# zju3dv/pats

Measured on AMD Instinct MI355X. Metric: image-pairs/sec (coarse+fine OT) on 640x480 MegaDepth; OT iters/sec per pair, higher is better.
Workload: dtype f32 (contractions: fp32 operands split into fp16 hi + lo, three exact-product MFMA passes, fp32 accumulate)

## Files before the change

### include/pats_amd.h

```cpp
#ifndef PATS_AMD_H
#define PATS_AMD_H

#include <stddef.h>
#include <stdint.h>

#ifdef __cplusplus
extern "C" {
#endif

typedef void* pats_stream_t;

enum {
    PATS_OK = 0,
    PATS_ERR_INVALID = 1,
    PATS_ERR_UNSUPPORTED = 2,
    PATS_ERR_LAUNCH = 3,
    PATS_ERR_NO_DEVICE = 4
};

enum { PATS_SINKHORN_AUTO = 0, PATS_SINKHORN_LOG = 1, PATS_SINKHORN_KERNEL = 2 };

const char* pats_version(void);
#define PATS_ABI_VERSION 8
int pats_abi_version(void);
const char* pats_last_error(void);
int pats_device_count(void);
int pats_set_sinkhorn_mode(int mode);
int pats_set_fine_fused(int on);

int pats_set_third_gather(int mode);

int pats_sinkhorn_fallbacks(int64_t* count, int reset);

int pats_sinkhorn_tail_solves(int64_t* count, int reset);

int pats_cost_f32(const float* d0, const float* d1, int64_t batch, int D, int n, int m, float* out,
                  pats_stream_t stream);

size_t pats_sinkhorn_workspace_bytes(int64_t batch, int M, int N);
int pats_sinkhorn_f32(const float* Z, int64_t batch, int M, int N, const float* log_mu,
                      const float* log_nu, int iters, float* out, void* workspace,
                      size_t workspace_bytes, pats_stream_t stream);

size_t pats_ot_workspace_bytes(int64_t batch, int M, int N);
int pats_log_optimal_transport_f32(const float* scores, int64_t batch, int m, int n,
                                   const float* alpha, const float* ns, int iters, float* Z,
                                   void* workspace, size_t workspace_bytes, pats_stream_t stream);

size_t pats_ot2_workspace_bytes(int64_t batch, int m, int n);
int pats_log_optimal_transport2_flags_f32(const float* scores, int64_t batch, int m, int n,
                                          const float* one, const float* ns, int iters, float bias_k,
                                          float* Z, uint8_t* col_nomatch, void* workspace,
                                          size_t workspace_bytes, pats_stream_t stream);
int pats_log_optimal_transport2_f32(const float* scores, int64_t batch, int m, int n,
                                    const float* one, const float* ns, int iters, float bias_k,
                                    float* Z, void* workspace, size_t workspace_bytes,
                                    pats_stream_t stream);

int pats_cost_ot_f32(const float* d0, const float* d1, int64_t batch, int D, int n, int m,
                     int variant, const float* scalar, const float* ns, int iters, float bias_k,
                     float* Z, void* workspace, size_t workspace_bytes, pats_stream_t stream);
size_t pats_cost_ot_workspace_bytes(int64_t batch, int D, int n, int m, int variant);
int pats_cost_ot_flags_f32(const float* d0, const float* d1, int64_t batch, int D, int n, int m,
// ... 589 lines not shown
```

### pats_amd/_lib.py

```python
import ctypes
import os

_HERE = os.path.dirname(os.path.abspath(__file__))
LIB_PATH = os.path.join(_HERE, "libpats_amd.so")
if os.environ.get("PATS_AMD_DIAG_LIB", "") not in ("", "0"):
    _sfx = os.environ["PATS_AMD_DIAG_LIB"]
    LIB_PATH = os.path.join(_HERE, "libpats_amd_diag%s.so" % ("" if _sfx == "1" else _sfx))

c_void_p, c_int, c_i64, c_f, c_size = (ctypes.c_void_p, ctypes.c_int, ctypes.c_int64, ctypes.c_float,
                                       ctypes.c_size_t)

ABI_VERSION = 8



class PairTable(ctypes.Structure):
    _fields_ = [("pairs", ctypes.c_int64), ("shape_host", c_void_p), ("cell_base_host", c_void_p), ("shape", c_void_p),
                ("cell_base", c_void_p), ("img_base", c_void_p)]


_TAB = ctypes.POINTER(PairTable)


class CropFormat(ctypes.Structure):
    _fields_ = [("dtype", ctypes.c_int32), ("layout", ctypes.c_int32), ("normalize", ctypes.c_int32),
                ("mean", ctypes.c_float * 3), ("std", ctypes.c_float * 3)]


_FMT = ctypes.POINTER(CropFormat)

_SCORE_ARGS = [c_void_p, c_void_p, c_void_p, c_void_p, c_i64, c_void_p, c_i64, c_i64, c_void_p, c_i64, c_void_p, c_void_p, c_int, c_f,
               c_void_p, c_void_p, c_void_p, c_void_p, c_void_p, c_void_p, c_size, c_void_p]
_ADAPTIVE_ARGS = [ctypes.c_double, c_int, c_int, c_i64, c_void_p, c_void_p]
_POLISH_ARGS = [c_void_p, c_void_p, c_void_p, c_void_p, c_i64, c_void_p, c_i64, c_i64, c_void_p, c_void_p, c_int, c_f, c_void_p, c_i64,
                c_void_p, c_int, c_void_p, c_void_p, c_void_p, c_void_p, c_void_p, c_void_p, c_void_p, c_size, c_void_p]

SIGNATURES = {
    "pats_version": (ctypes.c_char_p, []),
    "pats_abi_version": (c_int, []),
    "pats_last_error": (ctypes.c_char_p, []),
    "pats_device_count": (c_int, []),
    "pats_set_sinkhorn_mode": (c_int, [c_int]),
    "pats_set_fine_fused": (c_int, [c_int]),
    "pats_set_third_gather": (c_int, [c_int]),
    "pats_sinkhorn_fallbacks": (c_int, [ctypes.POINTER(ctypes.c_int64), c_int]),
    "pats_sinkhorn_tail_solves": (c_int, [ctypes.POINTER(ctypes.c_int64), c_int]),
    "pats_set_gnn_redo_mode": (c_int, [c_int]),
    "pats_gnn_overflows": (c_int, [ctypes.POINTER(ctypes.c_int64), c_int]),
    "pats_cost_f32": (c_int, [c_void_p, c_void_p, c_i64, c_int, c_int, c_int, c_void_p, c_void_p]),
    "pats_sinkhorn_workspace_bytes": (c_size, [c_i64, c_int, c_int]),
    "pats_sinkhorn_f32": (c_int, [c_void_p, c_i64, c_int, c_int, c_void_p, c_void_p, c_int, c_void_p,
                                  c_void_p, c_size, c_void_p]),
    "pats_ot_workspace_bytes": (c_size, [c_i64, c_int, c_int]),
    "pats_log_optimal_transport_f32": (c_int, [c_void_p, c_i64, c_int, c_int, c_void_p, c_void_p, c_int,
                                               c_void_p, c_void_p, c_size, c_void_p]),
    "pats_ot2_workspace_bytes": (c_size, [c_i64, c_int, c_int]),
    "pats_log_optimal_transport2_f32": (c_int, [c_void_p, c_i64, c_int, c_int, c_void_p, c_void_p, c_int,
                                                c_f, c_void_p, c_void_p, c_size, c_void_p]),
    "pats_cost_ot_f32": (c_int, [c_void_p, c_void_p, c_i64, c_int, c_int, c_int, c_int, c_void_p,
                                 c_void_p, c_int, c_f, c_void_p, c_void_p, c_size, c_void_p]),
    "pats_cost_ot_flags_f32": (c_int, [c_void_p, c_void_p, c_i64, c_int, c_int, c_int, c_int, c_void_p,
                                       c_void_p, c_int, c_f, c_void_p, c_void_p, c_void_p, c_size, c_void_p]),
    "pats_set_cost_ot_mid_event": (c_int, [c_void_p]),
    "pats_cost_ot_flags_counted_f32": (c_int, [c_void_p, c_void_p, c_i64, c_void_p, c_int, c_int, c_int, c_int, c_void_p,
                                               c_void_p, c_int, c_f, c_void_p, c_void_p, c_void_p, c_size, c_void_p]),
    "pats_iterative_expand_counted_f32": (c_int, [c_void_p, c_int, c_i64, c_void_p, c_int, c_int, c_void_p, c_void_p, c_int,
                                                  c_int, c_int, c_f, c_int, c_void_p, c_void_p, c_void_p,
                                                  c_void_p, c_void_p, c_void_p, c_void_p, c_void_p]),
    "pats_fine_descriptors_counted_f32": (c_int, [c_void_p, c_void_p, c_void_p, c_void_p, c_void_p, c_i64, c_void_p, c_int,
                                                  c_void_p, c_void_p]),
    "pats_log_optimal_transport2_flags_f32": (c_int, [c_void_p, c_i64, c_int, c_int, c_void_p, c_void_p, c_int,
                                                      c_f, c_void_p, c_void_p, c_void_p, c_size, c_void_p]),
    "pats_colmass_flags_f32": (c_int, [c_void_p, c_i64, c_int, c_int, c_void_p, c_void_p, c_void_p]),
    "pats_cost_ot_workspace_bytes": (c_size, [c_i64, c_int, c_int, c_int, c_int]),
    "pats_colmass_sqrt_f32": (c_int, [c_void_p, c_i64, c_int, c_int, c_void_p, c_void_p]),
    "pats_dustbin_bias_inplace_f32": (c_int, [c_void_p, c_i64, c_int, c_int, c_f, c_void_p]),
    "pats_exp_f32": (c_int, [c_void_p, c_i64, c_void_p, c_void_p]),
# ... 278 lines not shown
```

### pats_amd/csrc/expand.hip

```cpp
#include "common.hpp"
#include "third_device.hpp"

namespace pats {

struct ExpandArgs {
    const float* P;
    int input_is_log;
    int64_t rows_total;
    int M, N;
    const float* scalex;
    const float* scaley;
    int lim3, h, w;
    float lower_bound;
    int iter_num;
    float *whole_cost, *core_cost, *average_point, *x_scale, *y_scale;
    int64_t* bound;
    uint8_t* row_nomatch;
    const int64_t* live;
};

__device__ __forceinline__ float range_val(int d, int k) { return k <= d ? (float)k : 1e7f; }

__device__ __forceinline__ int clamp_seq(float f, int wh, int S) {
    return (f >= 0.f && f <= (float)(wh - 1)) ? (int)f : S;
}


template <bool SMALL>
__global__ void __launch_bounds__(256)
expand_kernel(ExpandArgs a) {
    extern __shared__ __attribute__((aligned(16))) float sm[];
    const int t = threadIdx.x & 15, slot = threadIdx.x >> 4;
    const int ROWS_PER_WG = blockDim.x >> 4;
    const int M = a.M, N = a.N, m = M - 1, n = N - 1;
    int64_t rows_total = a.rows_total;
    if (a.live) {
        const int64_t lv = *a.live * m;
        rows_total = lv < rows_total ? lv : rows_total;
        if ((int64_t)blockIdx.x * ROWS_PER_WG >= rows_total) return;
    }
    const int64_t gr_raw = (int64_t)blockIdx.x * ROWS_PER_WG + slot;
    const bool active = gr_raw < rows_total;
    const int64_t gr = active ? gr_raw : rows_total - 1;
    const int64_t b = gr / m;
    const int r = (int)(gr - b * m);
    const int ld = N + 3;
    float* prow = sm + (size_t)slot * ld;
    float* popp = sm + (size_t)ROWS_PER_WG * ld + (size_t)slot * ld;
    const float* Pb = a.P + b * (int64_t)M * N;
    const float* src = Pb + (int64_t)r * N;
    const float* oppsrc = Pb + (int64_t)(M - 1) * N;
    const float* sx = a.scalex + b * (int64_t)n;
    const float* sy = a.scaley + b * (int64_t)n;
    float fv = -INFINITY;
    int fi = 0x7fffffff;
    const int64_t g0 = (int64_t)blockIdx.x * ROWS_PER_WG;
    const int64_t glast = min(g0 + ROWS_PER_WG - 1, rows_total - 1);
    const int64_t b0 = g0 / m;
    const bool shared_opp = glast / m - b0 <= 1;
    if (shared_opp) {
        popp = sm + (size_t)ROWS_PER_WG * ld + (size_t)(b - b0) * ld;
        for (int e = threadIdx.x; e < 2 * N; e += blockDim.x) {
            const int which = e >= N, j = e - which * N;
            const int64_t bb = min(b0 + which, (int64_t)(rows_total - 1) / m);
            const float o = a.P[bb * (int64_t)M * N + (int64_t)(M - 1) * N + j];
            sm[(size_t)ROWS_PER_WG * ld + (size_t)which * ld + j] = a.input_is_log ? expf(o) : o;
        }
    }
    float bv = -INFINITY, bva = -INFINITY;
    int bi = 0x7fffffff, bia = 0x7fffffff;
    float rowsum = 0.f;
    for (int j = t; j < N; j += 16) {
        const float x0 = src[j];
        if (x0 > fv || fi == 0x7fffffff) { fv = x0; fi = j; }
        const float x = a.input_is_log ? expf(x0) : x0;
        prow[j] = x;
        rowsum += x;
        if (j < N - 1 && (x > bv || bi == 0x7fffffff)) { bv = x; bi = j; }
        if (x > bva || bia == 0x7fffffff) { bva = x; bia = j; }
        if (!shared_opp) {
            const float o = oppsrc[j];
            popp[j] = a.input_is_log ? expf(o) : o;
        }
    }
    if (a.row_nomatch) {
        row16_argmax(fv, fi);
        if (t == 0 && active) a.row_nomatch[gr] = fi == N - 1;
    }
    if (t == 0) { prow[N] = ZERO_F; popp[N] = ZERO_F; }
    wg_barrier();

    const int width = a.h > a.w ? a.h : a.w;
    const int height = (a.h * a.w) / width;
    const int wh = width * height, S = wh + 1;
    auto ES = [&](int idx) { return prow[idx]; };
    auto ESC = [&](int idx) { return idx < n ? sx[idx] * sy[idx] : ZERO_F; };
    auto EOPP = [&](int idx) { return popp[idx]; };

    row16_argmax(bv, bi);
    row16_argmax(bva, bia);
    const float the_scale = row16_sum(rowsum);
    const int max0 = bi;
    const bool if_nomatching = (bia == m);
    float last_nomatching = EOPP(max0);
    int up = max0 / a.lim3, down = up, left = max0 % a.lim3, right = left;
    int bd0 = 0, bd1 = 0, sb0 = 0, sb1 = 0;
    float last_sum = ES(max0);

    for (int it = 0; it < a.iter_num; ++it) {
        sb0 = bd0; sb1 = bd1;
        const float off[4] = {(float)(left + up * width - width),
                              (float)(left + down * width + width),
                              (float)(left + up * width - 1),
                              (float)(right + up * width + 1)};
        float es[4], nm[4], sc[4];
        float vcell[4];
        int scell[4];
#pragma unroll
        for (int d = 0; d < 4; ++d) {
            float e = 0.f, q = 0.f, c = 0.f;
            auto cell = [&](int k) {
                const float f = d < 2 ? range_val(sb1, k) + off[d] : range_val(sb0, k) * (float)width + off[d];
                const int s = clamp_seq(f, wh, S);
                const float v = ES(s);
                e += v;
                if (SMALL) { vcell[d] = v; scell[d] = s; }
                else {
                    q += (v > a.lower_bound) ? EOPP(s) : ZERO_F;
                    c += ESC(s);
                }
            };
            if (SMALL) { vcell[d] = 0.f; scell[d] = S; if (t < width) cell(t); }
            else for (int k = t; k < width; k += 16) cell(k);
            es[d] = row16_sum(e);
            if (!SMALL) { nm[d] = row16_sum(q); sc[d] = row16_sum(c); }
        }
        if (up == 0) es[0] = ZERO_F;
        if (down == height - 1) es[1] = ZERO_F;
        if (left == 0) es[2] = ZERO_F;
        if (right == width - 1) es[3] = ZERO_F;
        int arg = 0;
        float mx = es[0];
#pragma unroll
        for (int d = 1; d < 4; ++d)
            if (es[d] > mx) { mx = es[d]; arg = d; }
        float mnm;
        if (SMALL) {
            float v = vcell[0];
            int sidx = scell[0];
#pragma unroll
            for (int d = 1; d < 4; ++d)
                if (arg == d) { v = vcell[d]; sidx = scell[d]; }
            const float q = (t < width) ? ((v > a.lower_bound) ? EOPP(sidx) : ZERO_F) : 0.f;
            mnm = row16_sum(q);
        } else {
            mnm = nm[0];
#pragma unroll
            for (int d = 1; d < 4; ++d)
                if (arg == d) mnm = nm[d];
        }
        (void)sc;
        float add_sum = ZERO_F, add_nm = ZERO_F;
        if (mx > a.lower_bound) {
            up -= (arg == 0);
            down += (arg == 1);
            left -= (arg == 2);
            right += (arg == 3);
            add_sum = mx;
            add_nm = mnm;
        }
        bd0 = down - up;
        bd1 = right - left;
        last_sum = last_sum + add_sum;
        last_nomatching = last_nomatching + add_nm;
    }
    const bool if_core_exist = (bd0 > 1) && (bd1 > 1);

    float e4, s4;
    {
        const float eoff[4] = {(float)(left + up * width), (float)(left + down * width),
                               (float)(left + up * width), (float)(right + up * width)};
        float ed[4], sd[4];
#pragma unroll
        for (int d = 0; d < 4; ++d) {
            float e = 0.f, c = 0.f;
            auto cell = [&](int k) {
                const float f = d < 2 ? range_val(sb1, k) + eoff[d]
                                      : range_val(sb0, k) * (float)width + eoff[d];
                const int s = clamp_seq(f, wh, S);
                e += ES(s);
                c += ESC(s);
            };
            if (SMALL) { if (t < width) cell(t); }
            else for (int k = t; k < width; k += 16) cell(k);
            ed[d] = row16_sum(e);
            sd[d] = row16_sum(c);
        }
        e4 = (ed[0] + ed[1]) + (ed[2] + ed[3]);
        s4 = (sd[0] + sd[1]) + (sd[2] + sd[3]);
    }

    float wx = 0.f, wy = 0.f, sumx = 0.f, sumy = 0.f, ws = 0.f, so = 0.f;
    const int q16 = 16 / a.w, r16 = 16 - q16 * a.w;
    int pyi = t / a.w, pxi = t - pyi * a.w;
    const bool no_cell = up > (n - 1) / a.w || left > a.w - 1;
    for (int p = t; p < n; p += 16, pyi += q16, pxi += r16) {
        if (pxi >= a.w) { pxi -= a.w; ++pyi; }
        const bool crit = pyi >= up && pyi <= down && pxi >= left && pxi <= right;
        if (!__any(crit || no_cell)) continue;
        const float fx = sx[p], fy = sy[p];
        float ox = ZERO_F, oy = ZERO_F;
        if (crit) {
            const float root = sqrtf(prow[p] + 1e-7f);
            ox = root / fx;
            oy = root / fy;
        }
        wx += ox * (float)pxi;
        wy += oy * (float)pyi;
        sumx += ox;
        sumy += oy;
        const float o = ox * oy;
        ws += o * (fx * fy);
        so += o;
    }
    wx = row16_sum(wx); wy = row16_sum(wy); sumx = row16_sum(sumx); sumy = row16_sum(sumy);
    ws = row16_sum(ws); so = row16_sum(so);

    if (t == 0 && active) {
        const int corner[4] = {up * width + left, up * width + right, down * width + left,
                               down * width + right};
        float cps = 0.f, css = 0.f;
#pragma unroll
        for (int q = 0; q < 4; ++q) {
            int s = corner[q];
            if (!(s >= 0)) s = S;
            if (!(s <= wh - 1)) s = S;
            cps += ES(s);
            css += ESC(s);
        }
        const float core_scale_sum = the_scale - s4 + css;
        const float core_sum = last_sum - e4 + cps;
        a.core_cost[gr] = (if_core_exist && !if_nomatching)
                              ? fabsf((core_sum - core_scale_sum) / the_scale) : ZERO_F;
        a.whole_cost[gr] = if_nomatching ? ZERO_F
            : (fabsf(the_scale - last_sum) + last_nomatching / 4.0f) / the_scale;
        a.average_point[gr * 2 + 1] = wx / sumx + 0.5f;
        a.average_point[gr * 2 + 0] = wy / sumy + 0.5f;
        const float average_scale = sqrtf(ws / so);
        a.x_scale[gr] = 1.0f / (average_scale / 1.0f);
        a.y_scale[gr] = 1.0f / (average_scale * 1.0f);
        a.bound[gr * 4 + 0] = up;
        a.bound[gr * 4 + 1] = down;
        a.bound[gr * 4 + 2] = left;
        a.bound[gr * 4 + 3] = right;
    }
}

}

using namespace pats;

static int expand_impl(const float* P, int input_is_log, int64_t batch, int M, int N, const float* scalex, const float* scaley,
                       int lim3, int h, int w, float lower_bound, int iter_num, float* whole_cost, float* core_cost,
                       float* average_point, float* x_scale, float* y_scale, int64_t* bound, uint8_t* row_nomatch,
                       const int64_t* live, pats_stream_t stream);

extern "C" int pats_iterative_expand_f32(const float* P, int input_is_log, int64_t batch, int M,
                                         int N, const float* scalex, const float* scaley, int lim3,
                                         int h, int w, float lower_bound, int iter_num,
                                         float* whole_cost, float* core_cost, float* average_point,
                                         float* x_scale, float* y_scale, int64_t* bound,
                                         uint8_t* row_nomatch, pats_stream_t stream) {
    return expand_impl(P, input_is_log, batch, M, N, scalex, scaley, lim3, h, w, lower_bound, iter_num, whole_cost, core_cost,
                       average_point, x_scale, y_scale, bound, row_nomatch, nullptr, stream);
}

extern "C" int pats_iterative_expand_counted_f32(const float* P, int input_is_log, int64_t batch_cap, const int64_t* batch_dev,
                                                 int M, int N, const float* scalex, const float* scaley, int lim3, int h, int w,
                                                 float lower_bound, int iter_num, float* whole_cost, float* core_cost,
                                                 float* average_point, float* x_scale, float* y_scale, int64_t* bound,
                                                 uint8_t* row_nomatch, pats_stream_t stream) {
    PATS_REQUIRE(batch_dev, "iterative_expand_counted: null count");
    return expand_impl(P, input_is_log, batch_cap, M, N, scalex, scaley, lim3, h, w, lower_bound, iter_num, whole_cost, core_cost,
                       average_point, x_scale, y_scale, bound, row_nomatch, batch_dev, stream);
}

static int expand_impl(const float* P, int input_is_log, int64_t batch, int M, int N, const float* scalex, const float* scaley,
                       int lim3, int h, int w, float lower_bound, int iter_num, float* whole_cost, float* core_cost,
                       float* average_point, float* x_scale, float* y_scale, int64_t* bound, uint8_t* row_nomatch,
                       const int64_t* live, pats_stream_t stream) {
    PATS_REQUIRE(batch >= 0 && M > 1 && N > 1 && h > 0 && w > 0 && lim3 > 0 && iter_num >= 1,
                 "iterative_expand: bad argument");
    PATS_REQUIRE(h * w == N - 1, "iterative_expand: grid %dx%d does not match %d target columns", h,
                 w, N - 1);
    if (batch == 0) return PATS_OK;
    PATS_REQUIRE(P && scalex && scaley && whole_cost && core_cost && average_point && x_scale &&
                     y_scale && bound, "iterative_expand: null pointer");
    ExpandArgs a{P, input_is_log, batch * (int64_t)(M - 1), M, N, scalex, scaley, lim3, h, w,
                 lower_bound, iter_num, whole_cost, core_cost, average_point, x_scale, y_scale, bound, row_nomatch, live};
    int rows_per_wg = 16;
    size_t lds = 2 * (size_t)rows_per_wg * (size_t)(N + 3) * sizeof(float);
    if (lds > 48 * 1024) {
        rows_per_wg = 4;
        lds = 2 * (size_t)rows_per_wg * (size_t)(N + 3) * sizeof(float);
    }
    PATS_REQUIRE(lds <= 64 * 1024, "iterative_expand: N=%d too large", N);
    const int64_t blocks = ceil_div(a.rows_total, rows_per_wg);
    if (h <= 16 && w <= 16)
        hipLaunchKernelGGL(expand_kernel<true>, dim3((unsigned)blocks), dim3(16 * rows_per_wg), lds, as_stream(stream), a);
    else
        hipLaunchKernelGGL(expand_kernel<false>, dim3((unsigned)blocks), dim3(16 * rows_per_wg), lds, as_stream(stream), a);
    return check_launch("expand_kernel");
}
```

### pats_amd/csrc/host.cpp

```cpp
#include "common.hpp"
#include <stdlib.h>
#include "chunk_plan.hpp"

#include <atomic>
#include <mutex>
#include <string>

namespace pats {

static thread_local std::string g_last_error;

void set_error(const char* fmt, ...) {
    char buf[512];
    va_list ap;
    va_start(ap, fmt);
    vsnprintf(buf, sizeof(buf), fmt, ap);
    va_end(ap);
    g_last_error = buf;
}

int check_launch(const char* what) {
    hipError_t e = hipGetLastError();
    if (e != hipSuccess) {
        set_error("%s: %s", what, hipGetErrorString(e));
// ... 94 lines not shown

extern "C" int pats_stream_destroy(pats_stream_t stream) {
    if (stream && hipStreamDestroy(as_stream(stream)) != hipSuccess) return check_launch("hipStreamDestroy");
    return PATS_OK;
}

extern "C" const char* pats_last_error(void) { return g_last_error.c_str(); }

extern "C" int pats_device_count(void) {
    int n = 0;
    if (hipGetDeviceCount(&n) != hipSuccess) {
        (void)hipGetLastError();
        return 0;
    }
    return n;
}

extern "C" int pats_set_sinkhorn_mode(int mode) {
    const int prev = g_mode;
    if (mode == PATS_SINKHORN_AUTO || mode == PATS_SINKHORN_LOG || mode == PATS_SINKHORN_KERNEL)
        g_mode = mode;
    return prev;
}

static int g_fine_fused = env_switch("PATS_FINE_FUSED") && atoi(env_switch("PATS_FINE_FUSED")) != 0;
namespace pats { bool cost_f32_only() { static const bool on = [] { const char* e = env_switch("PATS_COST_F32"); return e && atoi(e) != 0; }(); return on; } }
namespace pats { bool fine_fused() { return g_fine_fused != 0; } }
extern "C" int pats_set_fine_fused(int on) {
    const int prev = g_fine_fused;
    g_fine_fused = on != 0;
    return prev;
}

extern "C" int pats_sinkhorn_fallbacks(int64_t* count, int reset) {
    PATS_REQUIRE(count, "sinkhorn_fallbacks: null pointer");
    unsigned long long* p = fallback_counter();
    PATS_REQUIRE(p, "sinkhorn_fallbacks: no counter on this device");
    unsigned long long v = 0;
    if (hipDeviceSynchronize() != hipSuccess) return check_launch("sinkhorn_fallbacks");
    if (hipMemcpy(&v, p, sizeof(v), hipMemcpyDeviceToHost) != hipSuccess) return check_launch("sinkhorn_fallbacks");
    if (reset && (hipMemset(p, 0, sizeof(v)) != hipSuccess || hipDeviceSynchronize() != hipSuccess))
        return check_launch("sinkhorn_fallbacks");
    *count = (int64_t)v;
    return PATS_OK;
}

extern "C" int pats_sinkhorn_tail_solves(int64_t* count, int reset) {
    PATS_REQUIRE(count, "sinkhorn_tail_solves: null pointer");
    unsigned long long* p = fallback_counter();
    PATS_REQUIRE(p, "sinkhorn_tail_solves: no counter on this device");
    unsigned long long v = 0;
    if (hipDeviceSynchronize() != hipSuccess) return check_launch("sinkhorn_tail_solves");
    if (hipMemcpy(&v, p + 1, sizeof(v), hipMemcpyDeviceToHost) != hipSuccess) return check_launch("sinkhorn_tail_solves");
    if (reset && (hipMemset(p + 1, 0, sizeof(v)) != hipSuccess || hipDeviceSynchronize() != hipSuccess))
        return check_launch("sinkhorn_tail_solves");
    *count = (int64_t)v;
    return PATS_OK;
}

namespace pats {
__global__ void split_patches_kernel(const int32_t* __restrict__ sc, int64_t pairs, int height, int width,
                                     int max_once_used, int64_t* __restrict__ second, int64_t* __restrict__ third,
                                     int32_t* __restrict__ cycle_num) {
    const int64_t i = (int64_t)blockIdx.x * blockDim.x + threadIdx.x;
    if (i >= pairs) return;
    const int64_t row = 2 * (int64_t)(height + 1);
// ... 26 lines not shown
```

### pats_amd/ops.py

```python
import collections
import ctypes
import math

import numpy as np
import torch

from . import _lib

_L = _lib.lib
_check = _lib.check
_L()


_raw_stream = getattr(torch._C, "_cuda_getCurrentRawStream", None)


def _stream():
    if _raw_stream is not None:
        return ctypes.c_void_p(_raw_stream(torch.cuda.current_device()))
    return ctypes.c_void_p(torch.cuda.current_stream().cuda_stream)


def _dev(t, name, dtype=torch.float32):
    if not isinstance(t, torch.Tensor):
# ... 79 lines not shown
def _workspace(nbytes, device):
    n = max(int(nbytes), 1)
    if not _WS_ON[0] or n > _WS_MAX or _raw_stream is None or torch.cuda.is_current_stream_capturing():
        return torch.empty(n, dtype=torch.uint8, device=device)
    key = (device.index, _raw_stream(torch.cuda.current_device()))
    t = _WS.get(key)
    if t is None or t.numel() < n:
        t = _WS[key] = torch.empty(min(_WS_MAX, max(2 * n, 1 << 20)), dtype=torch.uint8, device=device)
    return t


def _scalar_dev(x, device):
    if isinstance(x, torch.Tensor):
        return x.detach().reshape(1).to(device=device, dtype=torch.float32)
    return torch.full((1,), float(x), dtype=torch.float32, device=device)


def set_sinkhorn_mode(mode):
    names = {"auto": 0, "log": 1, "kernel": 2}
    prev = _L().pats_set_sinkhorn_mode(names[mode])
    return {v: k for k, v in names.items()}[prev]


def set_fine_fused(on):
    return bool(_L().pats_set_fine_fused(1 if on else 0))


def set_third_gather(mode):
    modes = {"tile": 0, "point": 1}
    if mode not in modes:
        raise ValueError("set_third_gather: mode must be 'tile' or 'point'")
    prev = _L().pats_set_third_gather(modes[mode])
    return {v: k for k, v in modes.items()}.get(prev, "tile")


def sinkhorn_fallbacks(reset=True):
    import ctypes
    n = ctypes.c_int64(0)
    rc = _L().pats_sinkhorn_fallbacks(ctypes.byref(n), 1 if reset else 0)
    if rc != 0:
        raise RuntimeError(_L().pats_last_error().decode())
    return int(n.value)


def sinkhorn_tail_solves(reset=True):
    n = ctypes.c_int64(0)
    _check(_L().pats_sinkhorn_tail_solves(ctypes.byref(n), 1 if reset else 0), "sinkhorn_tail_solves")
    return int(n.value)


def set_gnn_redo(mode):
    names = {"inline": 0, "deferred": 1}
    prev = _L().pats_set_gnn_redo_mode(names[mode])
    return {v: k for k, v in names.items()}[prev]


def gnn_overflows(reset=True):
    n = ctypes.c_int64(0)
    _check(_L().pats_gnn_overflows(ctypes.byref(n), 1 if reset else 0), "gnn_overflows")
    return bool(n.value)


def cost(mdesc0, mdesc1, out=None):
    (d0, d1), code = _descs_any([mdesc0, mdesc1], ["mdesc0", "mdesc1"])
    b, D, n = d0.shape
    if d1.shape[0] != b or d1.shape[1] != D:
# ... 2696 lines not shown
```

Baseline: 1957.

## Pack multiple expand rows per 16-lane group with non-finite redo pass

Adds a packed variant of the iterative expand kernel in which each row is handled by 4 or 8 lanes, each covering several columns, instead of 16 lanes. Each workgroup therefore processes 64 or 32 rows, and reductions use shorter DPP chains. Rows whose results are non-finite are flagged, and a second scan kernel recomputes them on the original 16-lane path. Packed mode is the default (4 lanes) when the expand window is small. The aim is to cut lanes wasted on narrow windows, at the cost of an extra redo launch and more registers per thread.

```diff
diff --git a/include/pats_amd.h b/include/pats_amd.h
--- a/include/pats_amd.h
+++ b/include/pats_amd.h
@@ -29,6 +29,8 @@
 int pats_set_fine_fused(int on);
 
 int pats_set_third_gather(int mode);
+
+int pats_set_expand_lanes(int lanes);
 
 int pats_sinkhorn_fallbacks(int64_t* count, int reset);
 
diff --git a/pats_amd/_lib.py b/pats_amd/_lib.py
--- a/pats_amd/_lib.py
+++ b/pats_amd/_lib.py
@@ -43,6 +43,7 @@
     "pats_set_sinkhorn_mode": (c_int, [c_int]),
     "pats_set_fine_fused": (c_int, [c_int]),
     "pats_set_third_gather": (c_int, [c_int]),
+    "pats_set_expand_lanes": (c_int, [c_int]),
     "pats_sinkhorn_fallbacks": (c_int, [ctypes.POINTER(ctypes.c_int64), c_int]),
     "pats_sinkhorn_tail_solves": (c_int, [ctypes.POINTER(ctypes.c_int64), c_int]),
     "pats_set_gnn_redo_mode": (c_int, [c_int]),
diff --git a/pats_amd/csrc/expand.hip b/pats_amd/csrc/expand.hip
--- a/pats_amd/csrc/expand.hip
+++ b/pats_amd/csrc/expand.hip
@@ -26,68 +26,108 @@
 }
 
 
-template <bool SMALL>
-__global__ void __launch_bounds__(256)
-expand_kernel(ExpandArgs a) {
-    extern __shared__ __attribute__((aligned(16))) float sm[];
-    const int t = threadIdx.x & 15, slot = threadIdx.x >> 4;
-    const int ROWS_PER_WG = blockDim.x >> 4;
+constexpr int64_t EXPAND_REDO = INT64_MIN;
+
+template <int LPP>
+__device__ __forceinline__ float packed_sum(const float (&x)[16 / LPP]) {
+    float v;
+    if constexpr (LPP == 8) v = x[0] + x[1];
+    else v = (x[0] + x[1]) + (x[2] + x[3]);
+    v += dpp_f<DPP_QUAD_XOR1>(v);
+    v += dpp_f<DPP_QUAD_XOR2>(v);
+    if constexpr (LPP == 8) v += dpp_f<DPP_ROW_HALF_MIRROR>(v);
+    return v;
+}
+template <int LPP>
+__device__ __forceinline__ void packed_argmax(float& v, int& i) {
+    argmax_step<DPP_QUAD_XOR1>(v, i);
+    argmax_step<DPP_QUAD_XOR2>(v, i);
+    if constexpr (LPP == 8) argmax_step<DPP_ROW_HALF_MIRROR>(v, i);
+}
+template <int CTRL>
+__device__ __forceinline__ float max_step(float v) {
+    const float ov = dpp_f<CTRL>(v);
+    return ov > v ? ov : v;
+}
+template <int LPP>
+__device__ __forceinline__ float packed_max(float v) {
+    v = max_step<DPP_QUAD_XOR1>(v);
+    v = max_step<DPP_QUAD_XOR2>(v);
+    if constexpr (LPP == 8) v = max_step<DPP_ROW_HALF_MIRROR>(v);
+    return v;
+}
+__device__ __forceinline__ int not_finite(float x) { return !(fabsf(x) < INFINITY); }
+
+template <int LPP>
+__device__ __forceinline__ void expand_packed(const ExpandArgs& a, float* sm) {
+    constexpr int CPL = 16 / LPP, PPW = 256 / LPP;
+    const int u = threadIdx.x & (LPP - 1), slot = threadIdx.x / LPP;
+    const int v0 = CPL * u;
     const int M = a.M, N = a.N, m = M - 1, n = N - 1;
     int64_t rows_total = a.rows_total;
     if (a.live) {
         const int64_t lv = *a.live * m;
         rows_total = lv < rows_total ? lv : rows_total;
-        if ((int64_t)blockIdx.x * ROWS_PER_WG >= rows_total) return;
-    }
-    const int64_t gr_raw = (int64_t)blockIdx.x * ROWS_PER_WG + slot;
+        if ((int64_t)blockIdx.x * PPW >= rows_total) return;
+    }
+    const int64_t g0 = (int64_t)blockIdx.x * PPW;
+    const int64_t gr_raw = g0 + slot;
     const bool active = gr_raw < rows_total;
     const int64_t gr = active ? gr_raw : rows_total - 1;
-    const int64_t b = gr / m;
+    const int64_t b = gr / m, b0 = g0 / m;
     const int r = (int)(gr - b * m);
     const int ld = N + 3;
     float* prow = sm + (size_t)slot * ld;
-    float* popp = sm + (size_t)ROWS_PER_WG * ld + (size_t)slot * ld;
-    const float* Pb = a.P + b * (int64_t)M * N;
-    const float* src = Pb + (int64_t)r * N;
-    const float* oppsrc = Pb + (int64_t)(M - 1) * N;
+    float* popp = sm + (size_t)PPW * ld + (size_t)(b - b0) * ld;
+    int* wave_nf = reinterpret_cast<int*>(sm + (size_t)(PPW + 2) * ld);
+    const float* src = a.P + b * (int64_t)M * N + (int64_t)r * N;
     const float* sx = a.scalex + b * (int64_t)n;
     const float* sy = a.scaley + b * (int64_t)n;
-    float fv = -INFINITY;
-    int fi = 0x7fffffff;
-    const int64_t g0 = (int64_t)blockIdx.x * ROWS_PER_WG;
-    const int64_t glast = min(g0 + ROWS_PER_WG - 1, rows_total - 1);
-    const int64_t b0 = g0 / m;
-    const bool shared_opp = glast / m - b0 <= 1;
-    if (shared_opp) {
-        popp = sm + (size_t)ROWS_PER_WG * ld + (size_t)(b - b0) * ld;
-        for (int e = threadIdx.x; e < 2 * N; e += blockDim.x) {
-            const int which = e >= N, j = e - which * N;
-            const int64_t bb = min(b0 + which, (int64_t)(rows_total - 1) / m);
-            const float o = a.P[bb * (int64_t)M * N + (int64_t)(M - 1) * N + j];
-            sm[(size_t)ROWS_PER_WG * ld + (size_t)which * ld + j] = a.input_is_log ? expf(o) : o;
-        }
-    }
-    float bv = -INFINITY, bva = -INFINITY;
-    int bi = 0x7fffffff, bia = 0x7fffffff;
-    float rowsum = 0.f;
-    for (int j = t; j < N; j += 16) {
+    {
+        const int64_t blast = (rows_total - 1) / m;
+        const float* opp0 = a.P + b0 * (int64_t)M * N + (int64_t)(M - 1) * N;
+        const float* opp1 = a.P + min(b0 + 1, blast) * (int64_t)M * N + (int64_t)(M - 1) * N;
+        float* st0 = sm + (size_t)PPW * ld;
+        bool bad0 = false, bad1 = false;
+#pragma unroll 1
+        for (int j = threadIdx.x; j < N; j += 256) {
+            const float o0 = a.input_is_log ? expf(opp0[j]) : opp0[j];
+            const float o1 = a.input_is_log ? expf(opp1[j]) : opp1[j];
+            st0[j] = o0;
+            st0[ld + j] = o1;
+            bad0 |= not_finite(o0);
+            bad1 |= not_finite(o1);
+        }
+        const int any0 = __any(bad0), any1 = __any(bad1);
+        if ((threadIdx.x & 63) == 0) { wave_nf[(threadIdx.x >> 6) * 2] = any0; wave_nf[(threadIdx.x >> 6) * 2 + 1] = any1; }
+    }
+    float bv = -INFINITY, inmax = -INFINITY;
+    int bi = 0x7fffffff;
+    float rowsum[CPL];
+#pragma unroll
+    for (int i = 0; i < CPL; ++i) rowsum[i] = 0.f;
+    auto stage = [&](int i, int j, bool real) {
         const float x0 = src[j];
-        if (x0 > fv || fi == 0x7fffffff) { fv = x0; fi = j; }
         const float x = a.input_is_log ? expf(x0) : x0;
         prow[j] = x;
-        rowsum += x;
-        if (j < N - 1 && (x > bv || bi == 0x7fffffff)) { bv = x; bi = j; }
-        if (x > bva || bia == 0x7fffffff) { bva = x; bia = j; }
-        if (!shared_opp) {
-            const float o = oppsrc[j];
-            popp[j] = a.input_is_log ? expf(o) : o;
-        }
-    }
-    if (a.row_nomatch) {
-        row16_argmax(fv, fi);
-        if (t == 0 && active) a.row_nomatch[gr] = fi == N - 1;
-    }
-    if (t == 0) { prow[N] = ZERO_F; popp[N] = ZERO_F; }
+        rowsum[i] += x;
+        if (real) {
+            inmax = x0 > inmax ? x0 : inmax;
+            if (x > bv) { bv = x; bi = j; }
+        }
+    };
+    const int full = n & ~15;
+    for (int j0 = v0; j0 < full; j0 += 16) {
+#pragma unroll
+        for (int i = 0; i < CPL; ++i) stage(i, j0 + i, true);
+    }
+#pragma unroll
+    for (int i = 0; i < CPL; ++i) {
+        const int j = full + v0 + i;
+        if (j < n) stage(i, j, true);
+        else if (j == n) stage(i, j, false);
+    }
+    if (u == 0) { prow[N] = ZERO_F; prow[N + 1] = 0.f; popp[N] = ZERO_F; popp[N + 1] = 0.f; }
     wg_barrier();
 
     const int width = a.h > a.w ? a.h : a.w;
@@ -97,43 +137,42 @@
     auto ESC = [&](int idx) { return idx < n ? sx[idx] * sy[idx] : ZERO_F; };
     auto EOPP = [&](int idx) { return popp[idx]; };
 
-    row16_argmax(bv, bi);
-    row16_argmax(bva, bia);
-    const float the_scale = row16_sum(rowsum);
-    const int max0 = bi;
-    const bool if_nomatching = (bia == m);
+    packed_argmax<LPP>(bv, bi);
+    const float the_scale = packed_sum<LPP>(rowsum);
+    int nf = not_finite(the_scale) | wave_nf[(int)(b - b0)] | wave_nf[2 + (int)(b - b0)] | wave_nf[4 + (int)(b - b0)] |
+                   wave_nf[6 + (int)(b - b0)];
+    if (a.row_nomatch) {
+        inmax = packed_max<LPP>(inmax);
+        if (u == 0 && active) a.row_nomatch[gr] = src[n] > inmax;
+    }
+    const int max0 = bi < n ? bi : 0;
+    const bool if_nomatching = (ES(n) > bv ? n : max0) == m;
     float last_nomatching = EOPP(max0);
     int up = max0 / a.lim3, down = up, left = max0 % a.lim3, right = left;
     int bd0 = 0, bd1 = 0, sb0 = 0, sb1 = 0;
     float last_sum = ES(max0);
 
+    bool inw[CPL];
+    int miss[CPL];
+#pragma unroll
+    for (int i = 0; i < CPL; ++i) { inw[i] = v0 + i < width; miss[i] = inw[i] ? S : N + 1; }
     for (int it = 0; it < a.iter_num; ++it) {
         sb0 = bd0; sb1 = bd1;
-        const float off[4] = {(float)(left + up * width - width),
-                              (float)(left + down * width + width),
-                              (float)(left + up * width - 1),
-                              (float)(right + up * width + 1)};
-        float es[4], nm[4], sc[4];
-        float vcell[4];
-        int scell[4];
+        const float off[4] = {(float)(left + up * width - width), (float)(left + down * width + width),
+                              (float)(left + up * width - 1), (float)(right + up * width + 1)};
+        float es[4];
+        int scell[4][CPL];
 #pragma unroll
         for (int d = 0; d < 4; ++d) {
-            float e = 0.f, q = 0.f, c = 0.f;
-            auto cell = [&](int k) {
+            float e[CPL];
+#pragma unroll
+            for (int i = 0; i < CPL; ++i) {
+                const int k = v0 + i;
                 const float f = d < 2 ? range_val(sb1, k) + off[d] : range_val(sb0, k) * (float)width + off[d];
-                const int s = clamp_seq(f, wh, S);
-                const float v = ES(s);
-                e += v;
-                if (SMALL) { vcell[d] = v; scell[d] = s; }
-                else {
-                    q += (v > a.lower_bound) ? EOPP(s) : ZERO_F;
-                    c += ESC(s);
-                }
-            };
-            if (SMALL) { vcell[d] = 0.f; scell[d] = S; if (t < width) cell(t); }
-            else for (int k = t; k < width; k += 16) cell(k);
-            es[d] = row16_sum(e);
-            if (!SMALL) { nm[d] = row16_sum(q); sc[d] = row16_sum(c); }
+                scell[d][i] = ((f >= 0.f) & (f <= (float)(wh - 1)) & inw[i]) ? (int)f : miss[i];
+                e[i] = 0.f + ES(scell[d][i]);
+            }
+            es[d] = packed_sum<LPP>(e);
         }
         if (up == 0) es[0] = ZERO_F;
         if (down == height - 1) es[1] = ZERO_F;
@@ -144,22 +183,16 @@
 #pragma unroll
         for (int d = 1; d < 4; ++d)
             if (es[d] > mx) { mx = es[d]; arg = d; }
-        float mnm;
-        if (SMALL) {
-            float v = vcell[0];
-            int sidx = scell[0];
+        float q[CPL];
+#pragma unroll
+        for (int i = 0; i < CPL; ++i) {
+            int sidx = scell[0][i];
 #pragma unroll
             for (int d = 1; d < 4; ++d)
-                if (arg == d) { v = vcell[d]; sidx = scell[d]; }
-            const float q = (t < width) ? ((v > a.lower_bound) ? EOPP(sidx) : ZERO_F) : 0.f;
-            mnm = row16_sum(q);
-        } else {
-            mnm = nm[0];
-#pragma unroll
-            for (int d = 1; d < 4; ++d)
-                if (arg == d) mnm = nm[d];
-        }
-        (void)sc;
+                if (arg == d) sidx = scell[d][i];
+            q[i] = EOPP(ES(sidx) > a.lower_bound ? sidx : miss[i]);
+        }
+        const float mnm = packed_sum<LPP>(q);
         float add_sum = ZERO_F, add_nm = ZERO_F;
         if (mx > a.lower_bound) {
             up -= (arg == 0);
@@ -183,52 +216,75 @@
         float ed[4], sd[4];
 #pragma unroll
         for (int d = 0; d < 4; ++d) {
-            float e = 0.f, c = 0.f;
-            auto cell = [&](int k) {
-                const float f = d < 2 ? range_val(sb1, k) + eoff[d]
-                                      : range_val(sb0, k) * (float)width + eoff[d];
+            float e[CPL], c[CPL];
+#pragma unroll
+            for (int i = 0; i < CPL; ++i) {
+                const int k = v0 + i;
+                const float f = d < 2 ? range_val(sb1, k) + eoff[d] : range_val(sb0, k) * (float)width + eoff[d];
                 const int s = clamp_seq(f, wh, S);
-                e += ES(s);
-                c += ESC(s);
-            };
-            if (SMALL) { if (t < width) cell(t); }
-            else for (int k = t; k < width; k += 16) cell(k);
-            ed[d] = row16_sum(e);
-            sd[d] = row16_sum(c);
+                const int sg = s < n ? s : 0;
+                const float esc = s < n ? sx[sg] * sy[sg] : ZERO_F;
+                e[i] = 0.f + ES(k < width ? s : N + 1);
+                c[i] = k < width ? 0.f + esc : 0.f;
+            }
+            ed[d] = packed_sum<LPP>(e);
+            sd[d] = packed_sum<LPP>(c);
         }
         e4 = (ed[0] + ed[1]) + (ed[2] + ed[3]);
         s4 = (sd[0] + sd[1]) + (sd[2] + sd[3]);
     }
 
-    float wx = 0.f, wy = 0.f, sumx = 0.f, sumy = 0.f, ws = 0.f, so = 0.f;
+    float wx[CPL], wy[CPL], sumx[CPL], sumy[CPL], ws[CPL], so[CPL];
+    int pyi[CPL], pxi[CPL];
     const int q16 = 16 / a.w, r16 = 16 - q16 * a.w;
-    int pyi = t / a.w, pxi = t - pyi * a.w;
+#pragma unroll
+    for (int i = 0; i < CPL; ++i) {
+        wx[i] = wy[i] = sumx[i] = sumy[i] = ws[i] = so[i] = 0.f;
+        pyi[i] = (v0 + i) / a.w;
+        pxi[i] = (v0 + i) - pyi[i] * a.w;
+    }
     const bool no_cell = up > (n - 1) / a.w || left > a.w - 1;
-    for (int p = t; p < n; p += 16, pyi += q16, pxi += r16) {
-        if (pxi >= a.w) { pxi -= a.w; ++pyi; }
-        const bool crit = pyi >= up && pyi <= down && pxi >= left && pxi <= right;
-        if (!__any(crit || no_cell)) continue;
-        const float fx = sx[p], fy = sy[p];
-        float ox = ZERO_F, oy = ZERO_F;
-        if (crit) {
-            const float root = sqrtf(prow[p] + 1e-7f);
-            ox = root / fx;
-            oy = root / fy;
-        }
-        wx += ox * (float)pxi;
-        wy += oy * (float)pyi;
-        sumx += ox;
-        sumy += oy;
-        const float o = ox * oy;
-        ws += o * (fx * fy);
-        so += o;
-    }
-    wx = row16_sum(wx); wy = row16_sum(wy); sumx = row16_sum(sumx); sumy = row16_sum(sumy);
-    ws = row16_sum(ws); so = row16_sum(so);
-
-    if (t == 0 && active) {
-        const int corner[4] = {up * width + left, up * width + right, down * width + left,
-                               down * width + right};
+    const int shared_lo = (threadIdx.x & 63) & ~(4 * LPP - 1);
+    const unsigned long long shared_mask = (4 * LPP == 64) ? ~0ull : ((1ull << (4 * LPP)) - 1ull);
+    for (int p0 = v0; p0 < n; p0 += 16) {
+        bool crit[CPL], reach = false;
+#pragma unroll
+        for (int i = 0; i < CPL; ++i) {
+            if (pxi[i] >= a.w) { pxi[i] -= a.w; ++pyi[i]; }
+            crit[i] = pyi[i] >= up && pyi[i] <= down && pxi[i] >= left && pxi[i] <= right;
+            reach |= (p0 + i < n) && (crit[i] || no_cell);
+        }
+        if (((__ballot(reach) >> shared_lo) & shared_mask) != 0ull) {
+#pragma unroll
+            for (int i = 0; i < CPL; ++i) {
+                const int p = p0 + i;
+                if (p < n) {
+                    const float fx = sx[p], fy = sy[p];
+                    float ox = ZERO_F, oy = ZERO_F;
+                    if (crit[i]) {
+                        const float root = sqrtf(prow[p] + 1e-7f);
+                        ox = root / fx;
+                        oy = root / fy;
+                    }
+                    wx[i] += ox * (float)pxi[i];
+                    wy[i] += oy * (float)pyi[i];
+                    sumx[i] += ox;
+                    sumy[i] += oy;
+                    const float o = ox * oy;
+                    ws[i] += o * (fx * fy);
+                    so[i] += o;
+                }
+            }
+        }
+#pragma unroll
+        for (int i = 0; i < CPL; ++i) { pyi[i] += q16; pxi[i] += r16; }
+    }
+    const float twx = packed_sum<LPP>(wx), twy = packed_sum<LPP>(wy), tsumx = packed_sum<LPP>(sumx), tsumy = packed_sum<LPP>(sumy);
+    const float tws = packed_sum<LPP>(ws), tso = packed_sum<LPP>(so);
+    nf |= not_finite(s4) | not_finite(twx) | not_finite(twy) | not_finite(tsumx) | not_finite(tsumy) | not_finite(tws) | not_finite(tso);
+
+    if (u == 0 && active) {
+        const int corner[4] = {up * width + left, up * width + right, down * width + left, down * width + right};
         float cps = 0.f, css = 0.f;
 #pragma unroll
         for (int q = 0; q < 4; ++q) {
@@ -240,25 +296,286 @@
         }
         const float core_scale_sum = the_scale - s4 + css;
         const float core_sum = last_sum - e4 + cps;
-        a.core_cost[gr] = (if_core_exist && !if_nomatching)
-                              ? fabsf((core_sum - core_scale_sum) / the_scale) : ZERO_F;
-        a.whole_cost[gr] = if_nomatching ? ZERO_F
-            : (fabsf(the_scale - last_sum) + last_nomatching / 4.0f) / the_scale;
-        a.average_point[gr * 2 + 1] = wx / sumx + 0.5f;
-        a.average_point[gr * 2 + 0] = wy / sumy + 0.5f;
-        const float average_scale = sqrtf(ws / so);
+        a.core_cost[gr] = (if_core_exist && !if_nomatching) ? fabsf((core_sum - core_scale_sum) / the_scale) : ZERO_F;
+        a.whole_cost[gr] = if_nomatching ? ZERO_F : (fabsf(the_scale - last_sum) + last_nomatching / 4.0f) / the_scale;
+        a.average_point[gr * 2 + 1] = twx / tsumx + 0.5f;
+        a.average_point[gr * 2 + 0] = twy / tsumy + 0.5f;
+        const float average_scale = sqrtf(tws / tso);
         a.x_scale[gr] = 1.0f / (average_scale / 1.0f);
         a.y_scale[gr] = 1.0f / (average_scale * 1.0f);
-        a.bound[gr * 4 + 0] = up;
+        a.bound[gr * 4 + 0] = nf ? EXPAND_REDO : (int64_t)up;
         a.bound[gr * 4 + 1] = down;
         a.bound[gr * 4 + 2] = left;
         a.bound[gr * 4 + 3] = right;
     }
 }
 
+template <bool SMALL, int LPP = 16, bool SCAN = false>
+__global__ void __launch_bounds__(256)
+expand_kernel(ExpandArgs a) {
+    extern __shared__ __attribute__((aligned(16))) float sm[];
+    if constexpr (LPP != 16) {
+        static_assert(SMALL && !SCAN && (LPP == 8 || LPP == 4), "packed lanes: SMALL grids, 8 or 4 lanes per patch");
+        expand_packed<LPP>(a, sm);
+        return;
+    }
+    [[maybe_unused]] unsigned todo = 0;
+    if constexpr (SCAN) {
+        int64_t rows_live = a.rows_total;
+        if (a.live) {
+            const int64_t lv = *a.live * (a.M - 1);
+            rows_live = lv < rows_live ? lv : rows_live;
+        }
+#pragma unroll
+        for (int q = 0; q < 4; ++q) {
+            const int64_t look = (int64_t)blockIdx.x * 256 + 64 * q + (threadIdx.x & 63);
+            const unsigned long long redo = __ballot(look < rows_live && a.bound[look * 4] == EXPAND_REDO);
+#pragma unroll
+            for (int s16 = 0; s16 < 4; ++s16)
+                if ((redo >> (16 * s16)) & 0xffffull) todo |= 1u << (4 * q + s16);
+        }
+    }
+    do {
+        unsigned blk = blockIdx.x;
+        if constexpr (SCAN) {
+            if (!todo) return;
+            blk = blockIdx.x * 16 + (__ffs((int)todo) - 1);
+            todo &= todo - 1;
+        }
+        const int t = threadIdx.x & 15, slot = threadIdx.x >> 4;
+        const int ROWS_PER_WG = blockDim.x >> 4;
+        const int M = a.M, N = a.N, m = M - 1, n = N - 1;
+        int64_t rows_total = a.rows_total;
+        if (a.live) {
+            const int64_t lv = *a.live * m;
+            rows_total = lv < rows_total ? lv : rows_total;
+            if ((int64_t)blk * ROWS_PER_WG >= rows_total) return;
+        }
+        const int64_t gr_raw = (int64_t)blk * ROWS_PER_WG + slot;
+        const bool active = gr_raw < rows_total;
+        const bool wanted = !SCAN || (active && a.bound[gr_raw * 4] == EXPAND_REDO);
+        const int64_t gr = active ? gr_raw : rows_total - 1;
+        const int64_t b = gr / m;
+        const int r = (int)(gr - b * m);
+        const int ld = N + 3;
+        float* prow = sm + (size_t)slot * ld;
+        float* popp = sm + (size_t)ROWS_PER_WG * ld + (size_t)slot * ld;
+        const float* Pb = a.P + b * (int64_t)M * N;
+        const float* src = Pb + (int64_t)r * N;
+        const float* oppsrc = Pb + (int64_t)(M - 1) * N;
+        const float* sx = a.scalex + b * (int64_t)n;
+        const float* sy = a.scaley + b * (int64_t)n;
+        float fv = -INFINITY;
+        int fi = 0x7fffffff;
+        const int64_t g0 = (int64_t)blk * ROWS_PER_WG;
+        const int64_t glast = min(g0 + ROWS_PER_WG - 1, rows_total - 1);
+        const int64_t b0 = g0 / m;
+        const bool shared_opp = glast / m - b0 <= 1;
+        if (shared_opp) {
+            popp = sm + (size_t)ROWS_PER_WG * ld + (size_t)(b - b0) * ld;
+            for (int e = threadIdx.x; e < 2 * N; e += blockDim.x) {
+                const int which = e >= N, j = e - which * N;
+                const int64_t bb = min(b0 + which, (int64_t)(rows_total - 1) / m);
+                const float o = a.P[bb * (int64_t)M * N + (int64_t)(M - 1) * N + j];
+                sm[(size_t)ROWS_PER_WG * ld + (size_t)which * ld + j] = a.input_is_log ? expf(o) : o;
+            }
+        }
+        float bv = -INFINITY, bva = -INFINITY;
+        int bi = 0x7fffffff, bia = 0x7fffffff;
+        float rowsum = 0.f;
+        for (int j = t; j < N; j += 16) {
+            const float x0 = src[j];
+            if (x0 > fv || fi == 0x7fffffff) { fv = x0; fi = j; }
+            const float x = a.input_is_log ? expf(x0) : x0;
+            prow[j] = x;
+            rowsum += x;
+            if (j < N - 1 && (x > bv || bi == 0x7fffffff)) { bv = x; bi = j; }
+            if (x > bva || bia == 0x7fffffff) { bva = x; bia = j; }
+            if (!shared_opp) {
+                const float o = oppsrc[j];
+                popp[j] = a.input_is_log ? expf(o) : o;
+            }
+        }
+        if (a.row_nomatch) {
+            row16_argmax(fv, fi);
+            if (t == 0 && active && wanted) a.row_nomatch[gr] = fi == N - 1;
+        }
+        if (t == 0) { prow[N] = ZERO_F; popp[N] = ZERO_F; }
+        wg_barrier();
+
+        const int width = a.h > a.w ? a.h : a.w;
+        const int height = (a.h * a.w) / width;
+        const int wh = width * height, S = wh + 1;
+        auto ES = [&](int idx) { return prow[idx]; };
+        auto ESC = [&](int idx) { return idx < n ? sx[idx] * sy[idx] : ZERO_F; };
+        auto EOPP = [&](int idx) { return popp[idx]; };
+
+        row16_argmax(bv, bi);
+        row16_argmax(bva, bia);
+        const float the_scale = row16_sum(rowsum);
+        const int max0 = bi;
+        const bool if_nomatching = (bia == m);
+        float last_nomatching = EOPP(max0);
+        int up = max0 / a.lim3, down = up, left = max0 % a.lim3, right = left;
+        int bd0 = 0, bd1 = 0, sb0 = 0, sb1 = 0;
+        float last_sum = ES(max0);
+
+        for (int it = 0; it < a.iter_num; ++it) {
+            sb0 = bd0; sb1 = bd1;
+            const float off[4] = {(float)(left + up * width - width),
+                                  (float)(left + down * width + width),
+                                  (float)(left + up * width - 1),
+                                  (float)(right + up * width + 1)};
+            float es[4], nm[4], sc[4];
+            float vcell[4];
+            int scell[4];
+    #pragma unroll
+            for (int d = 0; d < 4; ++d) {
+                float e = 0.f, q = 0.f, c = 0.f;
+                auto cell = [&](int k) {
+                    const float f = d < 2 ? range_val(sb1, k) + off[d] : range_val(sb0, k) * (float)width + off[d];
+                    const int s = clamp_seq(f, wh, S);
+                    const float v = ES(s);
+                    e += v;
+                    if (SMALL) { vcell[d] = v; scell[d] = s; }
+                    else {
+                        q += (v > a.lower_bound) ? EOPP(s) : ZERO_F;
+                        c += ESC(s);
+                    }
+                };
+                if (SMALL) { vcell[d] = 0.f; scell[d] = S; if (t < width) cell(t); }
+                else for (int k = t; k < width; k += 16) cell(k);
+                es[d] = row16_sum(e);
+                if (!SMALL) { nm[d] = row16_sum(q); sc[d] = row16_sum(c); }
+            }
+            if (up == 0) es[0] = ZERO_F;
+            if (down == height - 1) es[1] = ZERO_F;
+            if (left == 0) es[2] = ZERO_F;
+            if (right == width - 1) es[3] = ZERO_F;
+            int arg = 0;
+            float mx = es[0];
+    #pragma unroll
+            for (int d = 1; d < 4; ++d)
+                if (es[d] > mx) { mx = es[d]; arg = d; }
+            float mnm;
+            if (SMALL) {
+                float v = vcell[0];
+                int sidx = scell[0];
+    #pragma unroll
+                for (int d = 1; d < 4; ++d)
+                    if (arg == d) { v = vcell[d]; sidx = scell[d]; }
+                const float q = (t < width) ? ((v > a.lower_bound) ? EOPP(sidx) : ZERO_F) : 0.f;
+                mnm = row16_sum(q);
+            } else {
+                mnm = nm[0];
+    #pragma unroll
+                for (int d = 1; d < 4; ++d)
+                    if (arg == d) mnm = nm[d];
+            }
+            (void)sc;
+            float add_sum = ZERO_F, add_nm = ZERO_F;
+            if (mx > a.lower_bound) {
+                up -= (arg == 0);
+                down += (arg == 1);
+                left -= (arg == 2);
+                right += (arg == 3);
+                add_sum = mx;
+                add_nm = mnm;
+            }
+            bd0 = down - up;
+            bd1 = right - left;
+            last_sum = last_sum + add_sum;
+            last_nomatching = last_nomatching + add_nm;
+        }
+        const bool if_core_exist = (bd0 > 1) && (bd1 > 1);
+
+        float e4, s4;
+        {
+            const float eoff[4] = {(float)(left + up * width), (float)(left + down * width),
+                                   (float)(left + up * width), (float)(right + up * width)};
+            float ed[4], sd[4];
+    #pragma unroll
+            for (int d = 0; d < 4; ++d) {
+                float e = 0.f, c = 0.f;
+                auto cell = [&](int k) {
+                    const float f = d < 2 ? range_val(sb1, k) + eoff[d]
+                                          : range_val(sb0, k) * (float)width + eoff[d];
+                    const int s = clamp_seq(f, wh, S);
+                    e += ES(s);
+                    c += ESC(s);
+                };
+                if (SMALL) { if (t < width) cell(t); }
+                else for (int k = t; k < width; k += 16) cell(k);
+                ed[d] = row16_sum(e);
+                sd[d] = row16_sum(c);
+            }
+            e4 = (ed[0] + ed[1]) + (ed[2] + ed[3]);
+            s4 = (sd[0] + sd[1]) + (sd[2] + sd[3]);
+        }
+
+        float wx = 0.f, wy = 0.f, sumx = 0.f, sumy = 0.f, ws = 0.f, so = 0.f;
+        const int q16 = 16 / a.w, r16 = 16 - q16 * a.w;
+        int pyi = t / a.w, pxi = t - pyi * a.w;
+        const bool no_cell = up > (n - 1) / a.w || left > a.w - 1;
+        for (int p = t; p < n; p += 16, pyi += q16, pxi += r16) {
+            if (pxi >= a.w) { pxi -= a.w; ++pyi; }
+            const bool crit = pyi >= up && pyi <= down && pxi >= left && pxi <= right;
+            if (!__any(crit || no_cell)) continue;
+            const float fx = sx[p], fy = sy[p];
+            float ox = ZERO_F, oy = ZERO_F;
+            if (crit) {
+                const float root = sqrtf(prow[p] + 1e-7f);
+                ox = root / fx;
+                oy = root / fy;
+            }
+            wx += ox * (float)pxi;
+            wy += oy * (float)pyi;
+            sumx += ox;
+            sumy += oy;
+            const float o = ox * oy;
+            ws += o * (fx * fy);
+            so += o;
+        }
+        wx = row16_sum(wx); wy = row16_sum(wy); sumx = row16_sum(sumx); sumy = row16_sum(sumy);
+        ws = row16_sum(ws); so = row16_sum(so);
+
+        if (t == 0 && active && wanted) {
+            const int corner[4] = {up * width + left, up * width + right, down * width + left,
+                                   down * width + right};
+            float cps = 0.f, css = 0.f;
+    #pragma unroll
+            for (int q = 0; q < 4; ++q) {
+                int s = corner[q];
+                if (!(s >= 0)) s = S;
+                if (!(s <= wh - 1)) s = S;
+                cps += ES(s);
+                css += ESC(s);
+            }
+            const float core_scale_sum = the_scale - s4 + css;
+            const float core_sum = last_sum - e4 + cps;
+            a.core_cost[gr] = (if_core_exist && !if_nomatching)
+                                  ? fabsf((core_sum - core_scale_sum) / the_scale) : ZERO_F;
+            a.whole_cost[gr] = if_nomatching ? ZERO_F
+                : (fabsf(the_scale - last_sum) + last_nomatching / 4.0f) / the_scale;
+            a.average_point[gr * 2 + 1] = wx / sumx + 0.5f;
+            a.average_point[gr * 2 + 0] = wy / sumy + 0.5f;
+            const float average_scale = sqrtf(ws / so);
+            a.x_scale[gr] = 1.0f / (average_scale / 1.0f);
+            a.y_scale[gr] = 1.0f / (average_scale * 1.0f);
+            a.bound[gr * 4 + 0] = up;
+            a.bound[gr * 4 + 1] = down;
+            a.bound[gr * 4 + 2] = left;
+            a.bound[gr * 4 + 3] = right;
+        }
+        if constexpr (SCAN) wg_barrier();
+    } while (SCAN);
+}
+
 }
 
 using namespace pats;
+
+namespace pats { int expand_lanes(); }
 
 static int expand_impl(const float* P, int input_is_log, int64_t batch, int M, int N, const float* scalex, const float* scaley,
                        int lim3, int h, int w, float lower_bound, int iter_num, float* whole_cost, float* core_cost,
@@ -306,7 +623,16 @@
     }
     PATS_REQUIRE(lds <= 64 * 1024, "iterative_expand: N=%d too large", N);
     const int64_t blocks = ceil_div(a.rows_total, rows_per_wg);
-    if (h <= 16 && w <= 16)
+    const int lanes = expand_lanes();
+    const int packed_rows = 256 / lanes;
+    const size_t packed_lds = ((size_t)(packed_rows + 2) * (size_t)(N + 3) + 8) * sizeof(float);
+    if (h <= 16 && w <= 16 && lanes != 16 && M - 1 >= packed_rows && rows_per_wg == 16 && packed_lds <= 64 * 1024) {
+        const dim3 pgrid((unsigned)ceil_div(a.rows_total, packed_rows));
+        if (lanes == 8) hipLaunchKernelGGL((expand_kernel<true, 8>), pgrid, dim3(256), packed_lds, as_stream(stream), a);
+        else hipLaunchKernelGGL((expand_kernel<true, 4>), pgrid, dim3(256), packed_lds, as_stream(stream), a);
+        if (int rc = check_launch("expand_kernel (packed)")) return rc;
+        hipLaunchKernelGGL((expand_kernel<true, 16, true>), dim3((unsigned)ceil_div(a.rows_total, 256)), dim3(256), lds, as_stream(stream), a);
+    } else if (h <= 16 && w <= 16)
         hipLaunchKernelGGL(expand_kernel<true>, dim3((unsigned)blocks), dim3(16 * rows_per_wg), lds, as_stream(stream), a);
     else
         hipLaunchKernelGGL(expand_kernel<false>, dim3((unsigned)blocks), dim3(16 * rows_per_wg), lds, as_stream(stream), a);
diff --git a/pats_amd/csrc/host.cpp b/pats_amd/csrc/host.cpp
--- a/pats_amd/csrc/host.cpp
+++ b/pats_amd/csrc/host.cpp
@@ -150,6 +150,14 @@
     return prev;
 }
 
+static int g_expand_lanes = 4;
+namespace pats { int expand_lanes() { return g_expand_lanes; } }
+extern "C" int pats_set_expand_lanes(int lanes) {
+    const int prev = g_expand_lanes;
+    if (lanes == 16 || lanes == 8 || lanes == 4) g_expand_lanes = lanes;
+    return prev;
+}
+
 extern "C" int pats_sinkhorn_fallbacks(int64_t* count, int reset) {
     PATS_REQUIRE(count, "sinkhorn_fallbacks: null pointer");
     unsigned long long* p = fallback_counter();
diff --git a/pats_amd/ops.py b/pats_amd/ops.py
--- a/pats_amd/ops.py
+++ b/pats_amd/ops.py
@@ -135,6 +135,12 @@
         raise ValueError("set_third_gather: mode must be 'tile' or 'point'")
     prev = _L().pats_set_third_gather(modes[mode])
     return {v: k for k, v in modes.items()}.get(prev, "tile")
+
+
+def set_expand_lanes(lanes):
+    if lanes not in (16, 8, 4):
+        raise ValueError("set_expand_lanes: lanes must be 16, 8 or 4")
+    return int(_L().pats_set_expand_lanes(int(lanes)))
 
 
 def sinkhorn_fallbacks(reset=True):
```

New measurement: 1977 (median of 6 runs). 1.01x the previous value.
